# instaclustr/atsc

Hardware: AMD Instinct MI355X
Metric: Msamples/sec compressed (auto, e=5%) (higher is better)
Workload: dtype f64; 1 GPU; BASELINE.json configs[2] per GPU: 10,485,760 f64 samples, 40960 frames x 256, --compressor auto, e=5% (max_error=(float)5/100), classes C0-C4 cycled per 65536-sample block, inputs resident in HBM; the timed loop rotates over 5 different resident batches (series ids 0..4, batch b with the block -> class mapping shifted by 2 b); frames_per_gpu=40960, frame_len=256, encoded_bytes_rank0=3592754, parallelism=single GPU, GPU_MAX_HW_QUEUES=4

## Files before the change

atsc_amd/csrc/atsc_device.h:

```cpp
#pragma once
#include <hip/hip_runtime.h>
#include <stdint.h>

#include "../../include/atsc_hip.h"
#include "atsc_internal.h"

#include <map>
#include <mutex>
#include <utility>

namespace atsc {

#define DEVI __device__ __forceinline__
template <int W = 0>
DEVI uint32_t tid_now()
{
    uint32_t t = (W == 1) ? __builtin_amdgcn_mbcnt_hi(~0u, __builtin_amdgcn_mbcnt_lo(~0u, 0u)) : threadIdx.x;
    asm volatile("" : "+v"(t));
    return t;
}

inline hipError_t ensure_dyn_lds(const void *fn, uint32_t bytes)
{
    static std::mutex mu;
// ... 18 lines not shown
DEVI int32_t sat_i32(double x)
{
    if (x != x) return 0;
    if (x >= 2147483647.0) return INT32_MAX;
    if (x <= -2147483648.0) return INT32_MIN;
    return (int32_t)x;
}
DEVI int32_t sat_i16(double x)
{
    if (x != x) return 0;
    if (x >= 32767.0) return 32767;
    if (x <= -32768.0) return -32768;
    return (int32_t)x;
}
DEVI uint32_t sat_u8(double x)
{
    if (x != x) return 0;
    if (x >= 255.0) return 255;
    if (x <= 0.0) return 0;
    return (uint32_t)x;
}
DEVI uint32_t vlen(uint64_t v)
{
    return v < 251 ? 1u : v < (1ull << 16) ? 3u : v < (1ull << 32) ? 5u : 9u;
}
DEVI uint64_t zigzag(int64_t v)
{
    return v >= 0 ? ((uint64_t)v << 1) : ((~(uint64_t)v << 1) | 1ull);
}
DEVI uint32_t put_varint(uint8_t *p, uint64_t v)
{
    if (v < 251) {
        p[0] = (uint8_t)v;
        return 1;
    }
    uint32_t nb;
    if (v < (1ull << 16)) { p[0] = 251; nb = 2; }
    else if (v < (1ull << 32)) { p[0] = 252; nb = 4; }
    else { p[0] = 253; nb = 8; }
    for (uint32_t i = 0; i < nb; ++i) p[1 + i] = (uint8_t)(v >> (8 * i));
    return nb + 1;
}
DEVI void put_u32(uint8_t *p, uint32_t u)
{
    p[0] = (uint8_t)u; p[1] = (uint8_t)(u >> 8); p[2] = (uint8_t)(u >> 16); p[3] = (uint8_t)(u >> 24);
}
DEVI void put_f32(uint8_t *p, float f) { put_u32(p, __float_as_uint(f)); }
DEVI void put_u64(uint8_t *p, uint64_t u)
{
    put_u32(p, (uint32_t)u);
    put_u32(p + 4, (uint32_t)(u >> 32));
}
DEVI void put_f64(uint8_t *p, double d) { put_u64(p, (uint64_t)__double_as_longlong(d)); }

DEVI void split_n(double x, int64_t &ip, bool &frac_nz)
{
    const uint64_t bits = (uint64_t)__double_as_longlong(x);
    const bool neg = ((int64_t)bits) < 0;
    const int32_t exponent = (int32_t)((uint32_t)(bits >> 52) & 0x7ffu);
    const uint64_t mant_u = (bits & ((1ull << 52) - 1)) | (1ull << 52);
    const int64_t mant = neg ? -(int64_t)mant_u : (int64_t)mant_u;
    const int32_t shl = exponent + (64 - 53 - 1023 + 1);
    if (shl <= 0) {
        const int32_t shr = -shl;
        ip = 0;
        frac_nz = (shr < 64) ? ((((uint64_t)mant) >> shr) != 0) : false;
    } else if (shl < 64) {
        ip = mant >> (64 - shl);
        frac_nz = (((uint64_t)mant) << shl) != 0;
    } else if (shl < 128) {
        ip = (int64_t)(((uint64_t)mant) << (shl - 64));
        frac_nz = false;
    } else {
        ip = 0;
        frac_nz = false;
    }
}
DEVI uint32_t bitdepth_of(int64_t max_int, int64_t min_int)
{
    const int bd = max_int <= 255 ? 8 : max_int <= 32767 ? 16 : max_int <= 2147483647LL ? 32 : 64;
    const int bs = (min_int >= 0 && min_int <= 255) ? 8
                   : min_int >= -32768              ? 16
                   : min_int >= -2147483648LL       ? 32
                                                    : 64;
    const int m = bd > bs ? bd : bs;
    return m == 8 ? 3u : m == 16 ? 2u : m == 32 ? 1u : 0u;
}
DEVI uint32_t value_bytes(uint32_t bitdepth, double v)
{
    if (bitdepth == 3) return 1;
    if (bitdepth == 2) return vlen(zigzag((int64_t)sat_i16(v)));
    if (bitdepth == 1) return vlen(zigzag((int64_t)sat_i32(v)));
    return 8;
}
DEVI uint32_t put_value(uint8_t *p, uint32_t bitdepth, double v)
{
    if (bitdepth == 3) { p[0] = (uint8_t)sat_u8(v); return 1; }
    if (bitdepth == 2) return put_varint(p, zigzag((int64_t)sat_i16(v)));
    if (bitdepth == 1) return put_varint(p, zigzag((int64_t)sat_i32(v)));
    put_f64(p, v);
    return 8;
}

template <int CTRL, int ROWMASK>
DEVI uint32_t dpp_u32(uint32_t v)
{
    return (uint32_t)__builtin_amdgcn_update_dpp(0, (int)v, CTRL, ROWMASK, 0xf, false);
}
DEVI double lane_f64(double v, int l)
{
    const long long b = __double_as_longlong(v);
    const uint32_t lo = (uint32_t)__builtin_amdgcn_readlane((int)(uint32_t)b, l);
    const uint32_t hi = (uint32_t)__builtin_amdgcn_readlane((int)(uint32_t)((unsigned long long)b >> 32), l);
    return __longlong_as_double((long long)(((unsigned long long)hi << 32) | lo));
}
DEVI double wave_shr1_f64(double v)
{
    const long long b = __double_as_longlong(v);
    const int lo = (int)(uint32_t)b, hi = (int)(uint32_t)((unsigned long long)b >> 32);
    const uint32_t l2 = (uint32_t)__builtin_amdgcn_update_dpp(lo, lo, 0x138, 0xf, 0xf, false);
    const uint32_t h2 = (uint32_t)__builtin_amdgcn_update_dpp(hi, hi, 0x138, 0xf, 0xf, false);
    return __longlong_as_double((long long)(((unsigned long long)h2 << 32) | l2));
}
template <int CTRL, int ROWMASK>
DEVI uint32_t dpp_u32_keep(uint32_t v, uint32_t ident)
{
    return (uint32_t)__builtin_amdgcn_update_dpp((int)ident, (int)v, CTRL, ROWMASK, 0xf, false);
}
DEVI uint32_t wave_sum_u32(uint32_t v)
{
    v += dpp_u32<0xb1, 0xf>(v);
    v += dpp_u32<0x4e, 0xf>(v);
    v += dpp_u32<0x124, 0xf>(v);
    v += dpp_u32<0x128, 0xf>(v);
    v += dpp_u32<0x142, 0xa>(v);
    v += dpp_u32<0x143, 0xc>(v);
    return (uint32_t)__builtin_amdgcn_readlane((int)v, 63);
}
DEVI uint32_t wave_incl_scan_u32(uint32_t v)
{
    v += dpp_u32<0x111, 0xf>(v);
    v += dpp_u32<0x112, 0xf>(v);
    v += dpp_u32<0x114, 0xf>(v);
    v += dpp_u32<0x118, 0xf>(v);
    v += dpp_u32<0x142, 0xa>(v);
    v += dpp_u32<0x143, 0xc>(v);
    return v;
}
DEVI uint32_t wave_max_u32(uint32_t v)
{
    v = max(v, dpp_u32<0xb1, 0xf>(v));
    v = max(v, dpp_u32<0x4e, 0xf>(v));
    v = max(v, dpp_u32<0x124, 0xf>(v));
    v = max(v, dpp_u32<0x128, 0xf>(v));
// ... 717 lines not shown
```

atsc_amd/csrc/atsc_kernels.hip:

```cpp
#include <hip/hip_runtime.h>
#include <hip/hip_ext.h>
#include <stdint.h>
#include <stdlib.h>
#include <algorithm>
#include <string.h>

#include "atsc_device.h"

namespace atsc {

template <int W>
DEVI void fft_untangle(const DevPlan &P, const float2 *Z, float2 *out, const float2 *tw)
{
    constexpr int T = 64 * W;
    const uint32_t M = P.M;
    for (uint32_t k = tid_now<W>(); k <= M; k += T) {
        const float2 zk = Z[k == M ? 0 : k];
        const float2 zm = Z[k == 0 ? 0 : M - k];
        const float2 a = make_float2(zk.x + zm.x, zk.y - zm.y);
        const float2 b = make_float2(zk.x - zm.x, zk.y + zm.y);
        const float2 t = cmul_conj_tw(make_float2(b.y, -b.x), tw[k]);
        out[k] = make_float2(0.5f * a.x + 0.5f * t.x, 0.5f * a.y + 0.5f * t.y);
    }
    __syncthreads();
// ... 196 lines not shown
    __syncthreads();
}
template <int W>
DEVI void block_rank_sort_runs(uint32_t *rec, const double *xs, uint32_t count, uint32_t *tmp)
{
    constexpr uint32_t T = 64 * W;
    const uint32_t tid = tid_now<W>();
    uint32_t *rank = tmp + count;
    uint32_t p = 1;
    while (p < 16 && 2 * p * count <= T) p <<= 1;
    for (uint32_t i = tid; i < count; i += T) rank[i] = 0;
    __syncthreads();
    for (uint32_t w = tid; w < p * count; w += T) {
        const uint32_t i = w / p, q = w - i * p;
        const uint32_t ra = rec[i];
        const uint64_t ka = (uint64_t)__double_as_longlong(xs[ra & 0xffffu]);
        uint32_t r = 0;
        for (uint32_t j = q; j < count; j += p) {
            const uint32_t rb = rec[j];
            const uint64_t kb = (uint64_t)__double_as_longlong(xs[rb & 0xffffu]);
            r += (kb < ka || (kb == ka && rb < ra)) ? 1u : 0u;
        }
        if (p == 1) rank[i] = r;
        else if (r) atomicAdd(&rank[i], r);
    }
    __syncthreads();
    for (uint32_t i = tid; i < count; i += T) tmp[rank[i]] = rec[i];
    __syncthreads();
    for (uint32_t i = tid; i < count; i += T) rec[i] = tmp[i];
    __syncthreads();
}

#ifdef ATSC_STAMPS
__device__ unsigned long long g_phase_cyc[64 * 16];
__device__ unsigned long long g_frame_span[4 * 65536 * 3];
#define PH(i) do { if (FN != 0) { const long long now_ = clock64(); \
    if (tid == 0) atomicAdd(&ph_acc[i], (unsigned long long)(now_ - ph_t)); ph_t = clock64(); } } while (0)
#else
#define PH(i) do {} while (0)
#endif
template <int W, int SPL, bool IDW, int FN, bool LEAN_ = (FN != 0)>
__device__ __forceinline__ void compress_frame(
    const double *__restrict__ samples, const DevFrame *__restrict__ frames,
    const uint32_t *__restrict__ ids, const DevPlan *__restrict__ plans,
    const float2 *__restrict__ twpool, const KParams &prm, uint8_t *__restrict__ slots,
    DevResult *__restrict__ res, atsc_frame_diag *__restrict__ diag, const UniArgs &uni, const uint32_t bid)
{
    constexpr int T = 64 * W;
    constexpr bool FIX_ = FN != 0;
    extern __shared__ __attribute__((aligned(16))) unsigned char smem[];
    const uint32_t tid = tid_now<W>();
    uint32_t fid;
    DevFrame fr;
    const long long t_start = prm.cost ? clock64() : 0;
#ifdef ATSC_STAMPS
    __shared__ unsigned long long ph_acc[16];
    if (tid < 16) ph_acc[tid] = 0;
    __syncthreads();
    long long ph_t = clock64();
    const uint32_t span0 = 3u * 65536u * (((uint32_t)prm.debug_stop >> 24) & 3u);
    if (FN != 0 && tid == 0 && bid < 65536) {
        g_frame_span[span0 + 3 * bid] = wall_clock64();
        g_frame_span[span0 + 3 * bid + 2] = (unsigned long long)__builtin_amdgcn_s_getreg((31 << 11) | (0 << 6) | 4) |
                                           ((unsigned long long)__builtin_amdgcn_s_getreg((31 << 11) | (0 << 6) | 20) << 32);
    }
#endif
    if (FIX_ || uni.enabled) {
        const uint64_t dealt = (uint64_t)bid * uni.spread;
        const uint32_t r = uni.adaptive ? (uint32_t)__builtin_amdgcn_readfirstlane((int)(ids[bid] - uni.fid0))
                           : !uni.spread ? bid
                           : (dealt >> 32) == 0 ? spread_mod((uint32_t)dealt, uni.spread_m, uni.count)
                                                : (uint32_t)(dealt % uni.count);
        fid = uni.fid0 + r;
        fr.sample_off = uni.sample_off0 + (uint64_t)r * uni.n;
        fr.slot_off = uni.slot_off0 + (uint64_t)r * uni.slot_stride;
        fr.n = uni.n;
        fr.plan = uni.plan;
    } else {
        fid = ids[bid];
        fr = frames[fid];
    }
    typedef const __attribute__((address_space(4))) DevPlan PlanConst;
    PlanConst &P = *(PlanConst *)(plans + fr.plan);
#define P_GENERIC (*(const DevPlan *)&P)
    constexpr bool FIX = FN != 0;
    constexpr bool LEAN = LEAN_;
    static_assert(LEAN || !FIX, "fixed-length instantiations are lean");
    constexpr uint32_t cL = FIX ? cx_next_size(FIX ? FN : 1) : 0, cmf = (3 >= FN / 100) ? 3 : FN / 100;
    static_assert(!FIX || (FN >= 128 && cL <= 64 * W * SPL), "fixed-length instantiation");
    constexpr bool chalf = cL % 2 == 0;
    constexpr uint32_t cM = chalf ? cL / 2 : cL;
    const uint32_t n = FIX ? FN : P.n, L = FIX ? cL : P.L, pre = FIX ? (cL - FN) / 2 : P.pre;
    const uint32_t bins = FIX ? cL / 2 + 1 : P.bins;
    const uint32_t mf = FIX ? cmf : P.mf;
    constexpr uint32_t cdk1 = cmf / 2 > 1 ? cmf / 2 : 1, cdk2 = cmf / 10 > 1 ? cmf / 10 : 1;
    constexpr uint32_t ckcap = (cL / 2 + 1 < cmf + 17 * cdk1 + 5 * cdk2) ? cL / 2 + 1 : cmf + 17 * cdk1 + 5 * cdk2;
    const uint32_t dk1 = FIX ? cdk1 : P.dk1, dk2 = FIX ? cdk2 : P.dk2;
    constexpr EncLds lay = enc_lds(FIX ? FN : 1, FIX ? cL : 1, FIX ? cM : 1, false, ckcap, W == 1);
    const uint32_t o_xs = FIX ? lay.o_xs : P.o_xs, o_tw = FIX ? lay.o_tw : P.o_tw, o_ab = FIX ? lay.o_ab : P.o_ab;
    const uint32_t ab_half = FIX ? lay.ab_half : P.ab_half, ab_bytes = FIX ? lay.ab_bytes : P.ab_bytes;
    const uint32_t o_sel = FIX ? lay.o_sel : P.o_sel, o_aux = FIX ? lay.o_aux : P.o_aux, o_red = FIX ? lay.o_red : P.o_red;
    const uint32_t o_hist = FIX ? lay.o_hist : P.o_hist;
    const uint32_t kcap = FIX ? ckcap : P.kcap;

    double *xs = (double *)(smem + o_xs);
    float2 *tw = (float2 *)(smem + o_tw);
    unsigned char *AB = smem + o_ab;
    float2 *A = (float2 *)AB;
    float2 *B = (float2 *)(AB + ab_half);
    Sel *sel = (Sel *)(smem + o_sel);
    uint32_t *aux = (uint32_t *)(smem + o_aux);
    double *red = (double *)(smem + o_red);
    uint32_t *wsum = (W == 1) ? (uint32_t *)red : (uint32_t *)(red + 32);
    int parity = 0;

    uint8_t *out = slots + fr.slot_off;
    int mode = LEAN ? (int)ATSC_AUTO : prm.mode;
    const bool bounded = LEAN ? true : (prm.bounded != 0);

    constexpr bool REGSTAT = FIX && W == 1 && (FN == 256 || FN == 512);
    bool reg_stats = false;
    double rs_mn = 0.0, rs_mx = 0.0;
    uint32_t rs_frac = 0, rs_pk = 0;
    constexpr int TW4 = (SPL + 1) / 2;
    typedef float f32x4 __attribute__((ext_vector_type(4)));
    auto tw_copy = [&](const float2 *twp, const bool off_even) {
        if ((L & 1u) == 0 && off_even) {
            f32x4 r[TW4];
            walk_load<FIX ? (int)cL / 2 : 0, T, TW4>(r, (const f32x4 *)twp, tid, L >> 1);
            walk_store<FIX ? (int)cL / 2 : 0, T, TW4>(r, (f32x4 *)tw, tid, L >> 1);
        } else {
            float2 r[SPL];
            walk_load<FIX ? (int)cL : 0, T, SPL>(r, twp, tid, L);
            walk_store<FIX ? (int)cL : 0, T, SPL>(r, tw, tid, L);
        }
    };
    constexpr bool TWPRE = FIX && W == 1 && cL % 2 == 0 && FN != 128;
    bool tw_ready = false;
    f32x4 twr[TW4];
    if constexpr (TWPRE) {
        tw_ready = (uni.tw_off & 1ull) == 0;
        if (tw_ready) walk_load<(int)cL / 2, T, TW4>(twr, (const f32x4 *)(twpool + uni.tw_off), tid, cL / 2);
    }
#define TW_PUT() do { if constexpr (TWPRE) { \
        if (tw_ready) walk_store<(int)cL / 2, T, TW4>(twr, (f32x4 *)tw, tid, cL / 2); } } while (0)
    {
        const double *src = samples + fr.sample_off;
        if constexpr (REGSTAT) {
            if ((fr.sample_off & 1ull) == 0) {
                constexpr int NP = FN / 128;
                const double2 *src2 = (const double2 *)src;
                double2 *xs2 = (double2 *)xs;
                double2 v[NP];
#pragma unroll
                for (int m = 0; m < NP; ++m) v[m] = src2[tid + 64 * m];
                TW_PUT();
#pragma unroll
                for (int m = 0; m < NP; ++m) xs2[tid + 64 * m] = v[m];
                const double x0 = lane_f64(v[0].x, 0);
                rs_mn = x0;
                rs_mx = x0;
#pragma unroll
                for (int m = 0; m < NP; ++m) {
                    const double a = v[m].x, b = v[m].y;
                    rs_frac |= (frac_nonzero(a) || frac_nonzero(b)) ? 1u : 0u;
                    if (a > rs_mx) rs_mx = a;
                    if (a < rs_mn) rs_mn = a;
                    if (b > rs_mx) rs_mx = b;
                    if (b < rs_mn) rs_mn = b;
                    double left = wave_shr1_f64(b);
                    if (m > 0) {
                        const double wrap = lane_f64(v[m - 1].y, 63);
                        left = (tid == 0) ? wrap : left;
                    }
                    const uint32_t jx = 2u * (tid + 64u * (uint32_t)m);
                    if (jx == 0 || a != left) rs_pk += (vlen(jx) << 13) | 1u;
                    if (b != a) rs_pk += (vlen(jx + 1) << 13) | 1u;
                }
                reg_stats = true;
            }
        }
        if (reg_stats) {
        } else if (((fr.sample_off | n) & 1ull) == 0) {
            const double2 *src2 = (const double2 *)src;
            double2 *xs2 = (double2 *)xs;
            for_strided<FN / 2, T, (SPL + 1) / 2>(tid, n >> 1, [&](uint32_t j) { xs2[j] = src2[j]; });
        } else {
            for (uint32_t j = tid; j < n; j += T) xs[j] = src[j];
        }
        if (!reg_stats) TW_PUT();
    }
    __syncthreads();

    PH(0);
    double smin, smax;
    uint32_t bitdepth;
    uint32_t stat_pk = 0;
    bool stat_pk_done = false;
    {
        double mn, mx;
        uint32_t fr_any = 0;
        if (reg_stats) {
            mn = rs_mn; mx = rs_mx; fr_any = rs_frac;
        } else {
            const double x0 = xs[0];
            mn = x0; mx = x0;
            for_strided<FN, T, SPL>(tid, n, [&](uint32_t j) {
                const double v = xs[j];
                fr_any |= frac_nonzero(v) ? 1u : 0u;
                if (v > mx) mx = v;
                if (v < mn) mn = v;
                if constexpr (W > 1) {
                    const double b = xs[j ? j - 1 : 0];
                    if (j == 0 || v != b) stat_pk += (vlen(j) << 13) | 1u;
                }
            });
        }
        if constexpr (W > 1) {
            const BlockStats bs = block_stats4<W>(mn, mx, fr_any, stat_pk, red, wsum);
            mn = bs.mn; mx = bs.mx; fr_any = bs.frac; stat_pk = bs.pk;
            stat_pk_done = true;
        } else {
            mn = block_minmax_f64<W, true>(mn, red, parity);
            mx = block_minmax_f64<W, false>(mx, red, parity);
            fr_any = block_or_u32<W>(fr_any, red, parity);
        }
        smin = mn;
        smax = mx;
        if (mn == 0.0 || mx == 0.0) {
            uint32_t mni = 0xFFFFFFFFu, mxi = 0xFFFFFFFFu;
            for_strided<FN, T, SPL>(tid, n, [&](uint32_t j) {
                const double v = xs[j];
                if (v == mn) mni = min(mni, j);
                if (v == mx) mxi = min(mxi, j);
            });
            mni = block_min_u32<W>(mni, red, parity);
            mxi = block_min_u32<W>(mxi, red, parity);
            if (mni < n) smin = xs[mni];
            if (mxi < n) smax = xs[mxi];
        }
        int64_t maxi, mini;
        bool fz;
        split_n(smax, maxi, fz);
        split_n(smin, mini, fz);
        bitdepth = fr_any ? 0u : bitdepth_of(maxi, mini);
    }
    bool has_sub = false;
    if (tiny_range(smin, smax)) {
        uint32_t sb = 0;
        for_strided<FN, T, SPL>(tid, n, [&](uint32_t j) { sb |= __builtin_amdgcn_class(xs[j], 0x90) ? 1u : 0u; });
        has_sub = block_or_u32<W>(sb, red, parity) != 0;
    }

    PH(1);
    if (!LEAN && prm.debug_stop == 1) return;
    atsc_frame_diag dg;
    dg.fft_size = dg.poly_size = dg.rle_size = 0xFFFFFFFFu;
    dg.fft_trips = dg.fft_k = dg.poly_trips = dg.poly_step = 0;
    dg.poly_points = 0;
    dg.fft_err = dg.poly_err = 0.0;

    if (mode == ATSC_CONSTANT || (mode == ATSC_AUTO && (LEAN || !prm.trial) && smin == smax)) {
        if (tid == 0) {
            out[0] = 30;
            out[1] = (uint8_t)bitdepth;
            const uint32_t vb = put_value(out + 2, bitdepth, smin);
            res[fid].err = 0.0;
            res[fid].len = 2 + vb;
            res[fid].chosen = ATSC_CONSTANT;
            if (!LEAN && diag) diag[fid] = dg;
            if (prm.cost) prm.cost[fid] = (uint32_t)min((unsigned long long)(clock64() - t_start) >> 6, 0xFFFFFFFFull);
        }
        return;
    }

    if (mode == ATSC_NOOP) {
        for (uint32_t j = tid; j < n; j += T) aux[j] = vlen(zigzag(sat_i64(round(xs[j]))));
        __syncthreads();
        const uint32_t tot = block_excl_scan<W>(aux, n, wsum);
        const uint32_t hdr = 1 + vlen(n);
        for (uint32_t j = tid; j < n; j += T)
            put_varint(out + hdr + aux[j], zigzag(sat_i64(round(xs[j]))));
        if (tid == 0) {
            out[0] = 250;
            put_varint(out + 1, n);
            res[fid].err = 0.0;
            res[fid].len = hdr + tot;
            res[fid].chosen = ATSC_NOOP;
            if (!LEAN && diag) diag[fid] = dg;
        }
        return;
    }

    if (!LEAN && mode == ATSC_AUTO && prm.trial_res != nullptr && n >= prm.trial_min_n)
        mode = (int)prm.trial_res[fid].chosen;

    if (!LEAN && prm.debug_stop == 2) return;
    double g[SPL], inv[SPL];

    if (!LEAN && prm.debug_stop == 3) return;
    const bool run_fft = (mode == ATSC_AUTO || mode == ATSC_FFT);
    const bool run_poly = (mode == ATSC_AUTO || mode == ATSC_POLYNOMIAL || mode == ATSC_IDW);
    const bool run_rle = (mode == ATSC_AUTO || mode == ATSC_RLE);
    const bool idw = IDW && (mode == ATSC_IDW);
    const double me = prm.max_err;
    const bool prune = LEAN ? true : (mode == ATSC_AUTO) && (0.0 <= me);
    uint32_t best_size = 0xFFFFFFFFu;
    int best_owner = 3;
    auto can_win = [&](uint32_t size_lb, int owner) {
        return size_lb < best_size || (size_lb == best_size && owner < best_owner);
    };
    auto offer = [&](uint32_t size, int owner) {
        if (can_win(size, owner)) { best_size = size; best_owner = owner; }
    };
    uint32_t fft_k = 0, fft_size = 0xFFFFFFFFu, fft_trips = 0;
    double fft_err = 0.0;
    bool fft_done = false;
    const float mxf = (float)smax, mnf = (float)smin;
    uint32_t poly_step = 1, poly_K = 0, poly_size = 0xFFFFFFFFu, poly_trips = 0;
// ... 21 lines not shown
    uint32_t rle_size = 0xFFFFFFFFu, rle_R = 0, rle_D = 0, rle_ib = 0, rle_lb = 0xFFFFFFFFu;
    bool rle_sorted = false, rle_pending = false;
    bool rle_early = false;
    uint32_t *rrec_std = (uint32_t *)AB;
    uint32_t *rhp_std = rrec_std + n;
    uint32_t *rph_std = (uint32_t *)tw;
    auto run_key = [&](uint32_t rec) { return (uint64_t)__double_as_longlong(xs[rec & 0xffffu]); };
    auto rle_sort_and_group = [&](uint32_t *rrec, uint32_t *rhp, uint32_t *rph) {
        tw_ready = false;
        __syncthreads();
        for (uint32_t j = tid; j < n; j += T)
            aux[j] = (j + 1 >= n || xs[j + 1] != xs[j]) ? 1u : 0u;
        __syncthreads();
        const uint32_t R = block_excl_scan<W>(aux, n, wsum);
        uint32_t *ends = rhp;
        for (uint32_t j = tid; j < n; j += T)
            if (j + 1 >= n || xs[j + 1] != xs[j]) ends[aux[j]] = j;
        __syncthreads();
        for (uint32_t r = tid; r < R; r += T) {
            const uint32_t st = r ? ends[r - 1] + 1 : 0;
            rrec[r] = (st << 16) | ends[r];
        }
        __syncthreads();
        if (R <= 512 && 2 * R <= n + 2) {
            block_rank_sort_runs<W>(rrec, xs, R, aux);
        } else {
            uint32_t p2 = 1;
            while (p2 < R) p2 <<= 1;
            block_sort_runs<W>(rrec, xs, R, p2);
        }
        for (uint32_t i = tid; i < R; i += T)
            aux[i] = (i == 0 || run_key(rrec[i]) != run_key(rrec[i - 1])) ? 1u : 0u;
        __syncthreads();
        const uint32_t D = block_excl_scan<W>(aux, R, wsum);
        for (uint32_t i = tid; i < R; i += T)
            if (i == 0 || run_key(rrec[i]) != run_key(rrec[i - 1])) rhp[aux[i]] = i;
        if (tid == 0) rhp[D] = R;
        __syncthreads();
        uint32_t hb = 0;
        for (uint32_t gi = tid; gi < D; gi += T) {
            const uint32_t h0 = rhp[gi], h1 = rhp[gi + 1];
            const uint32_t b = value_bytes(bitdepth, xs[rrec[h0] & 0xffffu]) + vlen(h1 - h0);
            rph[gi] = b;
            hb += b;
        }
        __syncthreads();
        hb = block_sum_u32<W>(hb, red, parity);
        rle_R = R;
        rle_D = D;
        rle_size = 2 + vlen(D) + hb + rle_ib;
        rle_sorted = true;
    };
    bool rle_small = false;
    struct RleLane { uint32_t rec, cnt, hb, D, hb_total; bool head, live; };
    auto rle_small_build = [&]() {
        uint32_t *srt = (uint32_t *)AB, *ends = srt + 16;
        __syncthreads();
        const uint32_t C = (n + 63) >> 6, j0 = tid * C;
        uint32_t cnt = 0;
        for (uint32_t k = 0; k < C; ++k) {
            const uint32_t j = j0 + k;
            if (j < n && (j + 1 >= n || xs[j + 1] != xs[j])) ++cnt;
        }
        uint32_t pos = wave_incl_scan_u32(cnt) - cnt;
        for (uint32_t k = 0; k < C; ++k) {
            const uint32_t j = j0 + k;
            if (j < n && (j + 1 >= n || xs[j + 1] != xs[j])) ends[pos++] = j;
        }
        __syncthreads();
        const uint32_t R = rle_R;
        uint32_t rec = 0, klo = 0, khi = 0;
        if (tid < R) {
            const uint32_t e = ends[tid], st = tid ? ends[tid - 1] + 1 : 0;
            rec = (st << 16) | e;
            const uint64_t key = (uint64_t)__double_as_longlong(xs[e]);
            klo = (uint32_t)key;
            khi = (uint32_t)(key >> 32);
        }
        uint32_t rank = 0;
        for (uint32_t q = 0; q < R; ++q) {
            const uint32_t qlo = (uint32_t)__builtin_amdgcn_readlane((int)klo, (int)q);
            const uint32_t qhi = (uint32_t)__builtin_amdgcn_readlane((int)khi, (int)q);
            const bool less = qhi < khi || (qhi == khi && (qlo < klo || (qlo == klo && q < tid)));
            rank += less ? 1u : 0u;
        }
        if (tid < R) srt[rank] = rec;
        __syncthreads();
    };
    auto rle_small_group = [&]() -> RleLane {
        const uint32_t *srt = (const uint32_t *)AB;
        const uint32_t R = rle_R;
        RleLane g;
        g.live = tid < R;
        g.rec = g.live ? srt[tid] : 0u;
        const uint64_t key = g.live ? (uint64_t)__double_as_longlong(xs[g.rec & 0xffffu]) : 0ull;
        const uint32_t plo = dpp_u32<0x111, 0xf>((uint32_t)key), phi = dpp_u32<0x111, 0xf>((uint32_t)(key >> 32));
        g.head = g.live && (tid == 0 || plo != (uint32_t)key || phi != (uint32_t)(key >> 32));
        const uint64_t hm = __ballot(g.head);
        g.D = (uint32_t)__popcll(hm);
        const uint64_t after = (tid < 63) ? (hm >> (tid + 1)) : 0ull;
        const uint32_t next = after ? tid + 1 + (uint32_t)__builtin_ctzll(after) : R;
        g.cnt = next - tid;
        g.hb = g.head ? value_bytes(bitdepth, xs[g.rec & 0xffffu]) + vlen(g.cnt) : 0u;
        g.hb_total = wave_sum_u32(g.hb);
        return g;
    };
    if (run_rle) {
        uint32_t pk = 0;
        if (stat_pk_done) {
            pk = stat_pk;
        } else {
            if (reg_stats) {
                pk = rs_pk;
            } else {
                for_strided<FN, T, SPL>(tid, n, [&](uint32_t j) {
                    const double a = xs[j], b = xs[j ? j - 1 : 0];
                    if (j == 0 || a != b) pk += (vlen(j) << 13) | 1u;
                });
            }
            pk = block_sum_u32<W>(pk, red, parity);
        }
        rle_R = pk & 0x1fffu;
        rle_ib = pk >> 13;
        const uint32_t minval = (bitdepth == 0) ? 8u : 1u;
        rle_lb = 3 + rle_ib + (rle_R >= 2 ? 2u : 1u) * (minval + 1);
        if (W == 1 && rle_R <= 16 && ab_bytes >= 128) {
            rle_small_build();
            const RleLane g = rle_small_group();
            rle_D = g.D;
            rle_size = 2 + vlen(g.D) + g.hb_total + rle_ib;
            rle_small = true;
            rle_early = true;
            if (prune) offer(rle_size, 2);
        } else if (mode == ATSC_RLE) {
            rle_sort_and_group(rrec_std, rhp_std, rph_std);
            rle_sorted = true;
        } else if (rle_R <= 64 && 12 * rle_R + 16 <= ab_bytes) {
            uint32_t *e_rec = (uint32_t *)AB;
            rle_sort_and_group(e_rec, e_rec + rle_R, e_rec + 2 * rle_R + 1);
            rle_sorted = false;
            rle_early = true;
            if (prune) offer(rle_size, 2);
        } else {
            rle_pending = true;
        }
    }

    PH(2);
    if (!LEAN && prm.debug_stop == 10) return;
    if (!(prune && best_size < 19)) {
#pragma unroll
        for (int m = 0; m < SPL; ++m) {
            const uint32_t j = tid + m * T;
            int32_t i = (int32_t)j - (int32_t)pre;
            i = i < 0 ? 0 : (i >= (int32_t)n ? (int32_t)n - 1 : i);
            const double x = xs[i];
            g[m] = slice_in<FIX ? (int)cL : 0, T>(m, j, L) ? x : 1.0;
        }
        recip_abs_all<SPL>(g, inv);
#pragma unroll
        for (int m = 0; m < SPL; ++m)
            if (!slice_in<FIX ? (int)cL : 0, T>(m, tid + m * T, L)) inv[m] = 0.0;
    }

    PH(3);
    if (!LEAN && prm.debug_stop == 11) return;
    bool poly_first = false;
    if (prune && run_fft && run_poly && smax != smin) {
        poly_first = poly_payload_size(P.pstep[0], P.pK[0]) < 1 + 1 + 9 * min(mf, bins) + 8;
    }
    constexpr bool POLY2GO = W >= 16;
    double poly_cur = prm.max_err + 1.0;
    bool poly_paused = false;
    auto eval_poly = [&](const bool first_go) {
        if (run_poly) {
            bool poly_pruned = false;
            if (smax == smin) {
                poly_K = 0;
                poly_step = 1;
            } else if (!bounded) {
                poly_step = P.pstep[0];
// ... 433 lines not shown
                        }
                        used += cnt;
                    }
                }
                for (; used < K; ++used) {
                    uint32_t pos;
                    float2 z;
                    if (W == 1) {
                        pos = 0;
                        if (!heap_order) {
                            uint32_t lm = nb[0];
#pragma unroll
                            for (int m = 1; m < KPL; ++m) lm = max(lm, nb[m]);
                            const uint32_t wm = wave_max_u32(lm);
                            uint32_t mult = 0;
#pragma unroll
                            for (int m = KPL - 1; m >= 0; --m) {
                                const uint64_t bal = __ballot(nb[m] == wm);
                                mult += (uint32_t)__popcll(bal);
                                if (bal) pos = 64u * (uint32_t)m + (uint32_t)__builtin_ctzll(bal);
                            }
                            if (mult > 1) {
                                __syncthreads();
#pragma unroll
                                for (int m = 0; m < KPL; ++m) {
                                    const uint32_t k = tid + 64 * m;
                                    if (slice_in<FIX ? (int)cL / 2 + 1 : 0, 64>(m, k, bins)) {
                                        const float nrm = (float)sqrt((double)bre[m] * (double)bre[m] +
                                                                      (double)bim[m] * (double)bim[m]);
                                        keys[k] = ((uint64_t)__float_as_uint(nrm) << 32) | (uint64_t)k;
                                    }
                                }
                                __syncthreads();
                                hp_rebuild_parallel(keys, bins, tid, 64u);
                                hlen = bins;
                                for (uint32_t i = 0; i < used; ++i) (void)hp_pop(keys, hlen);
                                heap_order = true;
                            }
                        }
                        if (heap_order) pos = (uint32_t)(hp_pop(keys, hlen) & 0xffffffffu);
                        float zr = 0.0f, zi = 0.0f;
#pragma unroll
                        for (int m = 0; m < KPL; ++m) {
                            if (tid + 64 * m == pos) nb[m] = 0;
                            if ((pos >> 6) == (uint32_t)m) { zr = bre[m]; zi = bim[m]; }
                        }
                        z = make_float2(__uint_as_float(__builtin_amdgcn_readlane(__float_as_uint(zr), pos & 63)),
                                        __uint_as_float(__builtin_amdgcn_readlane(__float_as_uint(zi), pos & 63)));
                    } else {
                        pos = (uint32_t)(keys[heap_order ? bins - 1 - used : used] & 0xffffffffu);
                        z = spec[pos];
                    }
                    if (tid == 0) { sel[used].pos = pos; sel[used].re = z.x; sel[used].im = z.y; }
                    big += (pos >= 251) ? 1u : 0u;
                    const double cf = ((pos == 0 || 2 * pos == L) ? 1.0 : 2.0) * invL;
                    const float a = (float)(cf * (double)z.x);
                    const float b = (float)(cf * (double)z.y);
                    if (pos == 0) {
                        dc = a;
                    } else {
                        uint32_t idx = mod_magic(pos * tid, L, magicL);
                        const uint32_t stp = mod_magic(pos * (uint32_t)T, L, magicL);
#pragma unroll
                        for (int m = 0; m < SPL; ++m) {
                            const float2 w = tw[idx];
                            acc[m] = fmaf(a, w.x, acc[m]);
                            acc[m] = fmaf(-b, w.y, acc[m]);
                            idx += stp;
                            idx = min(idx, idx - L);
                        }
                    }
                }
                PH(7);
                if (!bounded) { cur = 0.0; break; }
                double s = 0.0;
                if (__builtin_expect(fast_clamp, 1)) {
#pragma unroll
                    for (int m = 0; m < SPL; ++m) {
                        const double x5 = (double)(acc[m] + dc) * 100000.0;
                        double o = div1e5(trunc(x5 + copysign(0.5, x5)));
                        o = fmin(fmax(o, mnd), mxd);
                        s += fabs(o - g[m]) * inv[m];
                    }
                } else {
#pragma unroll
                    for (int m = 0; m < SPL; ++m) {
                        if (tid + m * T < L) s += fft_term_slow(acc[m] + dc, mnd, mxd, g[m]);
                    }
                }
                s = block_sum_f64<W>(s, red, parity);
                cur = s * invL;
                PH(8);
                if (fft_trips <= 17) jump += dk1;
                else if (fft_trips <= 22) jump += dk2;
                else break;
            }
            fft_err = cur;
            fft_k = used;
            if (W > 1) {
                uint32_t b3 = 0;
                for (uint32_t i = tid; i < used; i += T) b3 += (sel[i].pos >= 251) ? 1u : 0u;
                big = block_sum_u32<W>(b3, red, parity);
            }
            fft_size = 1 + vlen(used) + 9 * used + 2 * big + 8;
            fft_done = !fft_pruned;
            __syncthreads();
        }
// ... 22 lines not shown
                if (j + 1 >= n || xs[j + 1] != xs[j]) {
                    const uint64_t key = (uint64_t)__double_as_longlong(xs[j]);
                    uint32_t h = __umulhi(((uint32_t)key ^ (uint32_t)(key >> 32)) * 0x9E3779B1u, H);
                    for (;;) {
                        const uint32_t old = atomicCAS(&tab[h], 0xFFFFFFFFu, j);
                        if (old == 0xFFFFFFFFu) { atomicAdd(&aux[j], 1u); ++dnew; break; }
                        if ((uint64_t)__double_as_longlong(xs[old]) == key) { atomicAdd(&aux[old], 1u); break; }
                        h = (h + 1 == H) ? 0 : h + 1;
                    }
                }
            }
            __syncthreads();
            uint32_t hb = 0;
            for (uint32_t j = tid; j < n; j += T)
                if (aux[j]) hb += value_bytes(bitdepth, xs[j]) + vlen(aux[j]);
            const uint32_t pk2 = block_sum_u32<W>((dnew << 18) | hb, red, parity);
            rle_D = pk2 >> 18;
            rle_size = 2 + vlen(rle_D) + (pk2 & 0x3ffffu) + rle_ib;
            if (prune) offer(rle_size, 2);
        } else {
            rle_size = rle_lb;
        }
    }
    dg.rle_size = rle_size;

    PH(11);
    if (!LEAN && prm.debug_stop == 8) return;
    int chosen;
    double chosen_err;
    if (mode == ATSC_AUTO) {
        if (prune) {
            chosen = best_owner == 0 ? ATSC_FFT : best_owner == 1 ? ATSC_POLYNOMIAL : ATSC_RLE;
        } else {
            chosen = ATSC_FFT;
            uint32_t bs = fft_size;
            if (poly_size < bs) { chosen = ATSC_POLYNOMIAL; bs = poly_size; }
            if (rle_size < bs) { chosen = ATSC_RLE; bs = rle_size; }
        }
        chosen_err = chosen == ATSC_FFT ? fft_err : chosen == ATSC_POLYNOMIAL ? poly_err : 0.0;
    } else {
        chosen = mode;
        chosen_err = mode == ATSC_FFT ? fft_err : (mode == ATSC_POLYNOMIAL || mode == ATSC_IDW) ? poly_err : 0.0;
    }

    uint32_t out_len = 0;
    if (!LEAN && prm.trial) {
        if (tid == 0) {
            res[fid].err = chosen_err;
            res[fid].len = 0;
            res[fid].chosen = (uint32_t)chosen;
        }
        return;
    }
    if (chosen == ATSC_FFT) {
        const uint32_t hdr = 1 + vlen(fft_k);
        for (uint32_t i = tid; i < fft_k; i += T) aux[i] = vlen(sel[i].pos) + 8;
        __syncthreads();
        const uint32_t body = block_excl_scan<W>(aux, fft_k, wsum);
        for (uint32_t i = tid; i < fft_k; i += T) {
            uint8_t *p = out + hdr + aux[i];
            p += put_varint(p, sel[i].pos & 0xffffu);
            put_f32(p, sel[i].re);
            put_f32(p + 4, sel[i].im);
        }
        if (tid == 0) {
            out[0] = 15;
            put_varint(out + 1, fft_k);
            put_f32(out + hdr + body, mxf);
            put_f32(out + hdr + body + 4, mnf);
        }
        out_len = hdr + body + 8;
    } else if (chosen == ATSC_POLYNOMIAL || chosen == ATSC_IDW) {
        const uint32_t hdr = 2 + vlen(poly_K);
        uint32_t body;
        if (bitdepth == 0 || bitdepth == 3) {
            const uint32_t vbytes = bitdepth == 0 ? 8u : 1u;
            body = poly_K * vbytes;
            for (uint32_t k = tid; k < poly_K; k += T) {
                const uint32_t t = (k == poly_K - 1) ? (n - 1) : k * poly_step;
                put_value(out + hdr + k * vbytes, bitdepth, xs[t]);
            }
        } else {
            for (uint32_t k = tid; k < poly_K; k += T) {
                const uint32_t t = (k == poly_K - 1) ? (n - 1) : k * poly_step;
                aux[k] = value_bytes(bitdepth, xs[t]);
            }
            __syncthreads();
            body = block_excl_scan<W>(aux, poly_K, wsum);
            for (uint32_t k = tid; k < poly_K; k += T) {
                const uint32_t t = (k == poly_K - 1) ? (n - 1) : k * poly_step;
                put_value(out + hdr + aux[k], bitdepth, xs[t]);
            }
        }
        if (tid == 0) {
            out[0] = idw ? 1 : 0;
            out[1] = (uint8_t)bitdepth;
            put_varint(out + 2, poly_K);
            put_f64(out + hdr + body, smin);
            put_f64(out + hdr + body + 8, smax);
            out[hdr + body + 16] = (uint8_t)poly_step;
        }
        out_len = hdr + body + 17;
    } else if (rle_small) {
        if (!rle_early) rle_small_build();
        const RleLane g = rle_small_group();
        const uint32_t hdr = 2 + vlen(g.D);
        const uint32_t st = g.rec >> 16, vl = g.live ? vlen(st) : 0u;
        const uint32_t vls = wave_incl_scan_u32(vl);
        const uint32_t hbs = wave_incl_scan_u32(g.hb);
        if (g.head) {
            uint8_t *p = out + hdr + (hbs - g.hb) + (vls - vl);
            p += put_value(p, bitdepth, xs[g.rec & 0xffffu]);
            put_varint(p, g.cnt);
        }
        if (g.live) put_varint(out + hdr + hbs + (vls - vl), st);
        if (tid == 0) {
            out[0] = 60;
            out[1] = (uint8_t)bitdepth;
            put_varint(out + 2, g.D);
        }
        out_len = hdr + g.hb_total + (uint32_t)__builtin_amdgcn_readlane((int)vls, 63);
    } else {
        uint32_t *rrec = rrec_std, *rhp = rhp_std, *rph = rph_std;
        if (rle_early) {
            rrec = (uint32_t *)AB;
            rhp = rrec + rle_R;
            rph = rrec + 2 * rle_R + 1;
        } else if (!rle_sorted) {
            rle_sort_and_group(rrec_std, rhp_std, rph_std);
        }
        const uint32_t R = rle_R, D = rle_D;
        const uint32_t hdr = 2 + vlen(D);
        for (uint32_t i = tid; i < R; i += T) {
            const uint32_t rec = rrec[i];
            const bool head = (i == 0 || run_key(rec) != run_key(rrec[i - 1]));
            aux[i] = (head ? 0x10000u : 0u) | vlen(rec >> 16);
        }
        __syncthreads();
        block_excl_scan<W>(aux, R, wsum);
        const uint32_t hb = block_excl_scan<W>(rph, D, wsum);
        uint32_t ibt = 0;
        for (uint32_t i = tid; i < R; i += T) {
            const uint32_t rec = rrec[i], st = rec >> 16;
            const bool head = (i == 0 || run_key(rec) != run_key(rrec[i - 1]));
            const uint32_t pk = aux[i], ps = pk & 0xffffu;
            const uint32_t gi = head ? (pk >> 16) : (pk >> 16) - 1;
            const uint32_t ghb = (gi + 1 < D ? rph[gi + 1] : hb);
            if (head) {
                uint8_t *p = out + hdr + rph[gi] + ps;
                p += put_value(p, bitdepth, xs[rec & 0xffffu]);
                put_varint(p, rhp[gi + 1] - rhp[gi]);
            }
            put_varint(out + hdr + ghb + ps, st);
            if (i == R - 1) ibt = ps + vlen(st);
        }
        ibt = block_sum_u32<W>(ibt, red, parity);
        if (tid == 0) {
            out[0] = 60;
            out[1] = (uint8_t)bitdepth;
            put_varint(out + 2, D);
        }
        out_len = hdr + hb + ibt;
    }
    PH(12);
#ifdef ATSC_STAMPS
    __syncthreads();
    if (FN != 0 && tid < 16) atomicAdd(&g_phase_cyc[(fid & 63u) * 16 + tid], ph_acc[tid]);
    if (FN != 0 && tid == 0 && bid < 65536) g_frame_span[span0 + 3 * bid + 1] = wall_clock64();
#endif
    if (tid == 0) {
        res[fid].err = chosen_err;
        res[fid].len = out_len;
        res[fid].chosen = (uint32_t)chosen;
        if (!LEAN && diag) diag[fid] = dg;
        if (prm.cost) prm.cost[fid] = (uint32_t)min((unsigned long long)(clock64() - t_start) >> 6, 0xFFFFFFFFull);
    }
}

template <int W, int SPL, bool IDW, int FN, bool LEAN_ = (FN != 0)>
__global__ __launch_bounds__(64 * W, (W == 1 && SPL <= 5 && !IDW) ? 6 : 1) void k_compress(
    const double *__restrict__ samples, const DevFrame *__restrict__ frames,
    const uint32_t *__restrict__ ids, const DevPlan *__restrict__ plans,
    const float2 *__restrict__ twpool, const KParams prm, uint8_t *__restrict__ slots,
    DevResult *__restrict__ res, atsc_frame_diag *__restrict__ diag, const UniArgs uni)
{
    compress_frame<W, SPL, IDW, FN, LEAN_>(samples, frames, ids, plans, twpool, prm, slots, res, diag, uni, blockIdx.x);
}

struct ClassSpans {
    uint32_t first[8], count[8];
    uint32_t n_spans, total;
};
DEVI uint32_t cost_bucket(uint32_t c)
{
    if (c == 0) return 0;
    const uint32_t msb = 31u - (uint32_t)__clz((int)c);
    const uint32_t sub = msb >= 2 ? (c >> (msb - 2)) & 3u : 0u;
    return min(63u, msb * 4u + sub);
}
DEVI uint32_t span_of(const ClassSpans &sp, uint32_t i)
{
    uint32_t c = 0;
    for (uint32_t k = 1; k < sp.n_spans; ++k)
        if (i >= sp.first[k]) c = k;
    return c;
}
__global__ __launch_bounds__(256) void k_cost_hist(const uint32_t *__restrict__ ids_src,
                                                   const uint32_t *cost, uint8_t *__restrict__ bkt,
                                                   uint32_t *__restrict__ hist, const ClassSpans sp)
{
    __shared__ uint32_t h[8 * 64];
    for (uint32_t k = threadIdx.x; k < 8 * 64; k += 256) h[k] = 0;
    __syncthreads();
    const uint32_t i = blockIdx.x * 256 + threadIdx.x;
    if (i < sp.total) {
// ... 443 lines not shown
```

Before: 107,400 Msamples/s.

## Stage encoded payload in LDS and flush with 16-byte stores; reuse run flags

```diff
diff --git a/atsc_amd/csrc/atsc_device.h b/atsc_amd/csrc/atsc_device.h
--- a/atsc_amd/csrc/atsc_device.h
+++ b/atsc_amd/csrc/atsc_device.h
@@ -94,6 +94,48 @@
     put_u32(p + 4, (uint32_t)(u >> 32));
 }
 DEVI void put_f64(uint8_t *p, double d) { put_u64(p, (uint64_t)__double_as_longlong(d)); }
+template <bool WIDE>
+DEVI void putx_u16(uint8_t *p, uint32_t u)
+{
+    if constexpr (WIDE) { const uint16_t h = (uint16_t)u; __builtin_memcpy(p, &h, 2); }
+    else { p[0] = (uint8_t)u; p[1] = (uint8_t)(u >> 8); }
+}
+template <bool WIDE>
+DEVI void putx_u32(uint8_t *p, uint32_t u)
+{
+    if constexpr (WIDE) __builtin_memcpy(p, &u, 4);
+    else put_u32(p, u);
+}
+template <bool WIDE>
+DEVI void putx_f32(uint8_t *p, float f) { putx_u32<WIDE>(p, __float_as_uint(f)); }
+template <bool WIDE>
+DEVI void putx_f32x2(uint8_t *p, float a, float b)
+{
+    if constexpr (WIDE) {
+        const uint64_t u = (uint64_t)__float_as_uint(a) | ((uint64_t)__float_as_uint(b) << 32);
+        __builtin_memcpy(p, &u, 8);
+    } else {
+        put_f32(p, a);
+        put_f32(p + 4, b);
+    }
+}
+template <bool WIDE>
+DEVI void putx_f64(uint8_t *p, double d)
+{
+    if constexpr (WIDE) __builtin_memcpy(p, &d, 8);
+    else put_f64(p, d);
+}
+template <bool WIDE>
+DEVI uint32_t putx_varint(uint8_t *p, uint64_t v)
+{
+    if constexpr (!WIDE) return put_varint(p, v);
+    if (v < 251) { p[0] = (uint8_t)v; return 1; }
+    if (v < (1ull << 16)) { p[0] = 251; putx_u16<true>(p + 1, (uint32_t)v); return 3; }
+    if (v < (1ull << 32)) { p[0] = 252; putx_u32<true>(p + 1, (uint32_t)v); return 5; }
+    p[0] = 253;
+    __builtin_memcpy(p + 1, &v, 8);
+    return 9;
+}
 
 DEVI void split_n(double x, int64_t &ip, bool &frac_nz)
 {
@@ -142,6 +184,19 @@
     if (bitdepth == 1) return put_varint(p, zigzag((int64_t)sat_i32(v)));
     put_f64(p, v);
     return 8;
+}
+template <bool WIDE>
+DEVI uint32_t putx_value(uint8_t *p, uint32_t bitdepth, double v)
+{
+    if (bitdepth == 3) { p[0] = (uint8_t)sat_u8(v); return 1; }
+    if (bitdepth == 2) return putx_varint<WIDE>(p, zigzag((int64_t)sat_i16(v)));
+    if (bitdepth == 1) return putx_varint<WIDE>(p, zigzag((int64_t)sat_i32(v)));
+    putx_f64<WIDE>(p, v);
+    return 8;
+}
+DEVI uint32_t mask_below(uint64_t m)
+{
+    return __builtin_amdgcn_mbcnt_hi((uint32_t)(m >> 32), __builtin_amdgcn_mbcnt_lo((uint32_t)m, 0u));
 }
 
 template <int CTRL, int ROWMASK>
diff --git a/atsc_amd/csrc/atsc_kernels.hip b/atsc_amd/csrc/atsc_kernels.hip
--- a/atsc_amd/csrc/atsc_kernels.hip
+++ b/atsc_amd/csrc/atsc_kernels.hip
@@ -272,7 +272,11 @@
     const uint32_t tid = tid_now<W>();
     uint32_t fid;
     DevFrame fr;
-    const long long t_start = prm.cost ? clock64() : 0;
+    constexpr bool ARGS1 = FIX_ && W == 1;
+    if constexpr (ARGS1)
+        asm volatile("" ::"s"(samples), "s"(ids), "s"(twpool), "s"(prm.cost), "s"(uni.adaptive), "s"(uni.fid0),
+                     "s"(uni.sample_off0), "s"(uni.spread), "s"(uni.count), "s"(uni.spread_m), "s"(uni.tw_off));
+    const long long t_start = (ARGS1 || prm.cost) ? clock64() : 0;
 #ifdef ATSC_STAMPS
     __shared__ unsigned long long ph_acc[16];
     if (tid < 16) ph_acc[tid] = 0;
@@ -287,12 +291,13 @@
 #endif
     if (FIX_ || uni.enabled) {
         const uint64_t dealt = (uint64_t)bid * uni.spread;
-        const uint32_t r = uni.adaptive ? (uint32_t)__builtin_amdgcn_readfirstlane((int)(ids[bid] - uni.fid0))
+        typedef const __attribute__((address_space(4))) uint32_t IdConst;
+        const uint32_t r = uni.adaptive ? (uint32_t)__builtin_amdgcn_readfirstlane((int)(*(IdConst *)(ids + bid) - uni.fid0))
                            : !uni.spread ? bid
                            : (dealt >> 32) == 0 ? spread_mod((uint32_t)dealt, uni.spread_m, uni.count)
                                                 : (uint32_t)(dealt % uni.count);
         fid = uni.fid0 + r;
-        fr.sample_off = uni.sample_off0 + (uint64_t)r * uni.n;
+        fr.sample_off = uni.sample_off0 + (uint64_t)r * (FIX_ ? (uint32_t)FN : uni.n);
         fr.slot_off = uni.slot_off0 + (uint64_t)r * uni.slot_stride;
         fr.n = uni.n;
         fr.plan = uni.plan;
@@ -322,6 +327,10 @@
     const uint32_t o_sel = FIX ? lay.o_sel : P.o_sel, o_aux = FIX ? lay.o_aux : P.o_aux, o_red = FIX ? lay.o_red : P.o_red;
     const uint32_t o_hist = FIX ? lay.o_hist : P.o_hist;
     const uint32_t kcap = FIX ? ckcap : P.kcap;
+    constexpr bool FFT1B = FIX && W == 1 && cL / 2 + 1 <= 251;
+    constexpr bool STAGE = FIX && W == 1 && FN != 128;
+    constexpr uint32_t STG_OFF = 128;
+    static_assert(!STAGE || STG_OFF + ((8u * FN + 22u + 15u) & ~15u) <= lay.ab_bytes, "payload staging fits in AB");
 
     double *xs = (double *)(smem + o_xs);
     float2 *tw = (float2 *)(smem + o_tw);
@@ -342,6 +351,8 @@
     bool reg_stats = false;
     double rs_mn = 0.0, rs_mx = 0.0;
     uint32_t rs_frac = 0, rs_pk = 0;
+    constexpr int RNP = REGSTAT ? FN / 128 : 1;
+    uint64_t rs_fa[RNP] = {}, rs_fb[RNP] = {};
     constexpr int TW4 = (SPL + 1) / 2;
     typedef float f32x4 __attribute__((ext_vector_type(4)));
     auto tw_copy = [&](const float2 *twp, const bool off_even) {
@@ -394,8 +405,11 @@
                         left = (tid == 0) ? wrap : left;
                     }
                     const uint32_t jx = 2u * (tid + 64u * (uint32_t)m);
-                    if (jx == 0 || a != left) rs_pk += (vlen(jx) << 13) | 1u;
-                    if (b != a) rs_pk += (vlen(jx + 1) << 13) | 1u;
+                    const bool sa = jx == 0 || a != left, sb = b != a;
+                    if (sa) rs_pk += (vlen(jx) << 13) | 1u;
+                    if (sb) rs_pk += (vlen(jx + 1) << 13) | 1u;
+                    rs_fa[m] = __ballot(sa);
+                    rs_fb[m] = __ballot(sb);
                 }
                 reg_stats = true;
             }
@@ -482,9 +496,8 @@
 
     if (mode == ATSC_CONSTANT || (mode == ATSC_AUTO && (LEAN || !prm.trial) && smin == smax)) {
         if (tid == 0) {
-            out[0] = 30;
-            out[1] = (uint8_t)bitdepth;
-            const uint32_t vb = put_value(out + 2, bitdepth, smin);
+            putx_u16<STAGE>(out, 30u | (bitdepth << 8));
+            const uint32_t vb = putx_value<STAGE>(out + 2, bitdepth, smin);
             res[fid].err = 0.0;
             res[fid].len = 2 + vb;
             res[fid].chosen = ATSC_CONSTANT;
@@ -612,30 +625,55 @@
         rle_sorted = true;
     };
     bool rle_small = false;
-    struct RleLane { uint32_t rec, cnt, hb, D, hb_total; bool head, live; };
-    auto rle_small_build = [&]() {
+    struct RleLane { uint32_t rec, cnt, hb, hbs, D, hb_total; bool head, live; };
+    constexpr bool RLEKEEP = REGSTAT;
+    uint32_t rle_rec = 0;
+    auto rle_small_build = [&](const bool from_flags) {
         uint32_t *srt = (uint32_t *)AB, *ends = srt + 16;
-        __syncthreads();
-        const uint32_t C = (n + 63) >> 6, j0 = tid * C;
-        uint32_t cnt = 0;
-        for (uint32_t k = 0; k < C; ++k) {
-            const uint32_t j = j0 + k;
-            if (j < n && (j + 1 >= n || xs[j + 1] != xs[j])) ++cnt;
-        }
-        uint32_t pos = wave_incl_scan_u32(cnt) - cnt;
-        for (uint32_t k = 0; k < C; ++k) {
-            const uint32_t j = j0 + k;
-            if (j < n && (j + 1 >= n || xs[j + 1] != xs[j])) ends[pos++] = j;
-        }
         __syncthreads();
         const uint32_t R = rle_R;
         uint32_t rec = 0, klo = 0, khi = 0;
-        if (tid < R) {
-            const uint32_t e = ends[tid], st = tid ? ends[tid - 1] + 1 : 0;
-            rec = (st << 16) | e;
-            const uint64_t key = (uint64_t)__double_as_longlong(xs[e]);
-            klo = (uint32_t)key;
-            khi = (uint32_t)(key >> 32);
+        if (REGSTAT && from_flags) {
+            uint32_t *starts = ends;
+            uint32_t base = 0;
+#pragma unroll
+            for (int m = 0; m < RNP; ++m) {
+                const uint64_t fa = rs_fa[m], fb = rs_fb[m];
+                const bool sa = ((fa >> tid) & 1ull) != 0, sb = ((fb >> tid) & 1ull) != 0;
+                const uint32_t at = base + mask_below(fa) + mask_below(fb);
+                const uint32_t jx = 2u * (tid + 64u * (uint32_t)m);
+                if (sa) starts[at] = jx;
+                if (sb) starts[at + (sa ? 1u : 0u)] = jx + 1;
+                base += (uint32_t)__popcll(fa) + (uint32_t)__popcll(fb);
+            }
+            __syncthreads();
+            if (tid < R) {
+                const uint32_t st = starts[tid], e = (tid + 1 < R) ? starts[tid + 1] - 1 : n - 1;
+                rec = (st << 16) | e;
+                const uint64_t key = (uint64_t)__double_as_longlong(xs[e]);
+                klo = (uint32_t)key;
+                khi = (uint32_t)(key >> 32);
+            }
+        } else {
+            const uint32_t C = (n + 63) >> 6, j0 = tid * C;
+            uint32_t cnt = 0;
+            for (uint32_t k = 0; k < C; ++k) {
+                const uint32_t j = j0 + k;
+                if (j < n && (j + 1 >= n || xs[j + 1] != xs[j])) ++cnt;
+            }
+            uint32_t pos = wave_incl_scan_u32(cnt) - cnt;
+            for (uint32_t k = 0; k < C; ++k) {
+                const uint32_t j = j0 + k;
+                if (j < n && (j + 1 >= n || xs[j + 1] != xs[j])) ends[pos++] = j;
+            }
+            __syncthreads();
+            if (tid < R) {
+                const uint32_t e = ends[tid], st = tid ? ends[tid - 1] + 1 : 0;
+                rec = (st << 16) | e;
+                const uint64_t key = (uint64_t)__double_as_longlong(xs[e]);
+                klo = (uint32_t)key;
+                khi = (uint32_t)(key >> 32);
+            }
         }
         uint32_t rank = 0;
         for (uint32_t q = 0; q < R; ++q) {
@@ -644,15 +682,20 @@
             const bool less = qhi < khi || (qhi == khi && (qlo < klo || (qlo == klo && q < tid)));
             rank += less ? 1u : 0u;
         }
-        if (tid < R) srt[rank] = rec;
-        __syncthreads();
+        if constexpr (RLEKEEP) {
+            const uint32_t got = (uint32_t)__builtin_amdgcn_ds_permute((int)(((tid < R) ? rank : 63u) << 2), (int)rec);
+            rle_rec = (tid < R) ? got : 0u;
+        } else {
+            if (tid < R) srt[rank] = rec;
+            __syncthreads();
+        }
     };
-    auto rle_small_group = [&]() -> RleLane {
+    auto rle_small_group = [&](const bool kept) -> RleLane {
         const uint32_t *srt = (const uint32_t *)AB;
         const uint32_t R = rle_R;
         RleLane g;
         g.live = tid < R;
-        g.rec = g.live ? srt[tid] : 0u;
+        g.rec = kept ? rle_rec : g.live ? srt[tid] : 0u;
         const uint64_t key = g.live ? (uint64_t)__double_as_longlong(xs[g.rec & 0xffffu]) : 0ull;
         const uint32_t plo = dpp_u32<0x111, 0xf>((uint32_t)key), phi = dpp_u32<0x111, 0xf>((uint32_t)(key >> 32));
         g.head = g.live && (tid == 0 || plo != (uint32_t)key || phi != (uint32_t)(key >> 32));
@@ -662,7 +705,8 @@
         const uint32_t next = after ? tid + 1 + (uint32_t)__builtin_ctzll(after) : R;
         g.cnt = next - tid;
         g.hb = g.head ? value_bytes(bitdepth, xs[g.rec & 0xffffu]) + vlen(g.cnt) : 0u;
-        g.hb_total = wave_sum_u32(g.hb);
+        g.hbs = wave_incl_scan_u32(g.hb);
+        g.hb_total = (uint32_t)__builtin_amdgcn_readlane((int)g.hbs, 63);
         return g;
     };
     if (run_rle) {
@@ -685,8 +729,8 @@
         const uint32_t minval = (bitdepth == 0) ? 8u : 1u;
         rle_lb = 3 + rle_ib + (rle_R >= 2 ? 2u : 1u) * (minval + 1);
         if (W == 1 && rle_R <= 16 && ab_bytes >= 128) {
-            rle_small_build();
-            const RleLane g = rle_small_group();
+            rle_small_build(reg_stats);
+            const RleLane g = rle_small_group(RLEKEEP);
             rle_D = g.D;
             rle_size = 2 + vlen(g.D) + g.hb_total + rle_ib;
             rle_small = true;
@@ -1226,7 +1270,7 @@
                         z = spec[pos];
                     }
                     if (tid == 0) { sel[used].pos = pos; sel[used].re = z.x; sel[used].im = z.y; }
-                    big += (pos >= 251) ? 1u : 0u;
+                    if constexpr (!FFT1B) big += (pos >= 251) ? 1u : 0u;
                     const double cf = ((pos == 0 || 2 * pos == L) ? 1.0 : 2.0) * invL;
                     const float a = (float)(cf * (double)z.x);
                     const float b = (float)(cf * (double)z.y);
@@ -1355,22 +1399,32 @@
         }
         return;
     }
+    uint8_t *const ob = STAGE ? AB + STG_OFF : out;
+    bool staged = STAGE;
     if (chosen == ATSC_FFT) {
         const uint32_t hdr = 1 + vlen(fft_k);
-        for (uint32_t i = tid; i < fft_k; i += T) aux[i] = vlen(sel[i].pos) + 8;
-        __syncthreads();
-        const uint32_t body = block_excl_scan<W>(aux, fft_k, wsum);
-        for (uint32_t i = tid; i < fft_k; i += T) {
-            uint8_t *p = out + hdr + aux[i];
-            p += put_varint(p, sel[i].pos & 0xffffu);
-            put_f32(p, sel[i].re);
-            put_f32(p + 4, sel[i].im);
+        uint32_t body;
+        if constexpr (FFT1B) {
+            body = 9 * fft_k;
+            for (uint32_t i = tid; i < fft_k; i += T) {
+                uint8_t *p = ob + hdr + 9 * i;
+                p[0] = (uint8_t)sel[i].pos;
+                putx_f32x2<STAGE>(p + 1, sel[i].re, sel[i].im);
+            }
+        } else {
+            for (uint32_t i = tid; i < fft_k; i += T) aux[i] = vlen(sel[i].pos) + 8;
+            __syncthreads();
+            body = block_excl_scan<W>(aux, fft_k, wsum);
+            for (uint32_t i = tid; i < fft_k; i += T) {
+                uint8_t *p = ob + hdr + aux[i];
+                p += putx_varint<STAGE>(p, sel[i].pos & 0xffffu);
+                putx_f32x2<STAGE>(p, sel[i].re, sel[i].im);
+            }
         }
         if (tid == 0) {
-            out[0] = 15;
-            put_varint(out + 1, fft_k);
-            put_f32(out + hdr + body, mxf);
-            put_f32(out + hdr + body + 4, mnf);
+            ob[0] = 15;
+            putx_varint<STAGE>(ob + 1, fft_k);
+            putx_f32x2<STAGE>(ob + hdr + body, mxf, mnf);
         }
         out_len = hdr + body + 8;
     } else if (chosen == ATSC_POLYNOMIAL || chosen == ATSC_IDW) {
@@ -1381,8 +1435,16 @@
             body = poly_K * vbytes;
             for (uint32_t k = tid; k < poly_K; k += T) {
                 const uint32_t t = (k == poly_K - 1) ? (n - 1) : k * poly_step;
-                put_value(out + hdr + k * vbytes, bitdepth, xs[t]);
-            }
+                putx_value<STAGE>(ob + hdr + k * vbytes, bitdepth, xs[t]);
+            }
+        } else if (STAGE && poly_K <= 64) {
+            const bool on = tid < poly_K;
+            const uint32_t t = !on ? 0u : (tid == poly_K - 1) ? (n - 1) : tid * poly_step;
+            const double v = xs[t];
+            const uint32_t vb = on ? value_bytes(bitdepth, v) : 0u;
+            const uint32_t in = wave_incl_scan_u32(vb);
+            body = (uint32_t)__builtin_amdgcn_readlane((int)in, 63);
+            if (on) putx_value<STAGE>(ob + hdr + (in - vb), bitdepth, v);
         } else {
             for (uint32_t k = tid; k < poly_K; k += T) {
                 const uint32_t t = (k == poly_K - 1) ? (n - 1) : k * poly_step;
@@ -1392,38 +1454,37 @@
             body = block_excl_scan<W>(aux, poly_K, wsum);
             for (uint32_t k = tid; k < poly_K; k += T) {
                 const uint32_t t = (k == poly_K - 1) ? (n - 1) : k * poly_step;
-                put_value(out + hdr + aux[k], bitdepth, xs[t]);
+                putx_value<STAGE>(ob + hdr + aux[k], bitdepth, xs[t]);
             }
         }
         if (tid == 0) {
-            out[0] = idw ? 1 : 0;
-            out[1] = (uint8_t)bitdepth;
-            put_varint(out + 2, poly_K);
-            put_f64(out + hdr + body, smin);
-            put_f64(out + hdr + body + 8, smax);
-            out[hdr + body + 16] = (uint8_t)poly_step;
+            putx_u16<STAGE>(ob, (idw ? 1u : 0u) | (bitdepth << 8));
+            putx_varint<STAGE>(ob + 2, poly_K);
+            putx_f64<STAGE>(ob + hdr + body, smin);
+            putx_f64<STAGE>(ob + hdr + body + 8, smax);
+            ob[hdr + body + 16] = (uint8_t)poly_step;
         }
         out_len = hdr + body + 17;
     } else if (rle_small) {
-        if (!rle_early) rle_small_build();
-        const RleLane g = rle_small_group();
+        if (!RLEKEEP && !rle_early) rle_small_build(false);
+        const RleLane g = rle_small_group(RLEKEEP);
         const uint32_t hdr = 2 + vlen(g.D);
         const uint32_t st = g.rec >> 16, vl = g.live ? vlen(st) : 0u;
         const uint32_t vls = wave_incl_scan_u32(vl);
-        const uint32_t hbs = wave_incl_scan_u32(g.hb);
+        const uint32_t hbs = g.hbs;
         if (g.head) {
-            uint8_t *p = out + hdr + (hbs - g.hb) + (vls - vl);
-            p += put_value(p, bitdepth, xs[g.rec & 0xffffu]);
-            put_varint(p, g.cnt);
-        }
-        if (g.live) put_varint(out + hdr + hbs + (vls - vl), st);
+            uint8_t *p = ob + hdr + (hbs - g.hb) + (vls - vl);
+            p += putx_value<STAGE>(p, bitdepth, xs[g.rec & 0xffffu]);
+            putx_varint<STAGE>(p, g.cnt);
+        }
+        if (g.live) putx_varint<STAGE>(ob + hdr + hbs + (vls - vl), st);
         if (tid == 0) {
-            out[0] = 60;
-            out[1] = (uint8_t)bitdepth;
-            put_varint(out + 2, g.D);
+            putx_u16<STAGE>(ob, 60u | (bitdepth << 8));
+            putx_varint<STAGE>(ob + 2, g.D);
         }
         out_len = hdr + g.hb_total + (uint32_t)__builtin_amdgcn_readlane((int)vls, 63);
     } else {
+        staged = false;
         uint32_t *rrec = rrec_std, *rhp = rhp_std, *rph = rph_std;
         if (rle_early) {
             rrec = (uint32_t *)AB;
@@ -1464,6 +1525,15 @@
             put_varint(out + 2, D);
         }
         out_len = hdr + hb + ibt;
+    }
+    if constexpr (STAGE) {
+        if (staged) {
+            typedef uint32_t u32x4 __attribute__((ext_vector_type(4)));
+            __syncthreads();
+            const u32x4 *s16 = (const u32x4 *)(AB + STG_OFF);
+            u32x4 *d16 = (u32x4 *)out;
+            for (uint32_t c = tid; c < (out_len + 15u) >> 4; c += T) d16[c] = s16[c];
+        }
     }
     PH(12);
 #ifdef ATSC_STAMPS
```

Result: faster. 108,900 Msamples/s, median of 6 (+1.4%).
